# QinZiwen/VisionX-SLAM

Measured on AMD Instinct MI355X. Metric: ms/frame (feature-extract+match + BA solve), 640×480, 50 KF / 20k pts, lower is better.
Workload: dtype u8/i32 (FAST, pyramid, BRIEF), f32 (Harris, blur, angle), f64 (BA)

## Files before the change

### visionx-slam_amd/csrc/ba.hip

```cpp
#include <algorithm>
#include <cstddef>
#include <cstdlib>
#include <chrono>
#include <cmath>
#include <type_traits>
#include <cstring>
#include <unordered_map>
#include <unordered_set>
#include <vector>

#include "vx_internal.hpp"
#include "vx_ktrace.hpp"
#include "ba_common.hpp"
#include "ba_plan.hpp"
#include "dmap.hpp"

namespace vx {
namespace {

using namespace vx::ba;

constexpr int kPoseBlock = kBaPoseBlock;
constexpr int kNTerms = 29;
constexpr int kStride = kBaStride;
// ... 815 lines not shown
        double h[9];
        const D3 PO{lpos[3 * orec.y], lpos[3 * orec.y + 1], lpos[3 * orec.y + 2]};
        const bool ok = obs_terms<kFT <= kFTSmall>(a, PO, orec.x, ouv, kslot, kLdsStride, kslot + 8, kLdsStride,
                                                   kslot + 17, kLdsStride, h);
#pragma unroll
        for (int j = 0; j < 9; ++j) terms[j * kFT + tid] = h[j];
        tcount[tid] = (has_o && ok) ? 1 : 0;
        __syncthreads();
        if (own) {
            double hs[9] = {0, 0, 0, 0, 0, 0, 0, 0, 0};
            int obs = 0;
            for (int r = run.x; r < run.y; ++r) {
#pragma unroll
                for (int j = 0; j < 9; ++j) hs[j] += terms[j * kFT + r];
                obs += tcount[r];
            }
            asm volatile("" : "+v"(lslot));
            PL = lm_update(a, lslot, PL, hs, obs);
            if (kEcopy) f.lpos[base + tid] = make_double4(PL.x, PL.y, PL.z, 0.0);
            lpos[3 * tid] = PL.x;
            lpos[3 * tid + 1] = PL.y;
            lpos[3 * tid + 2] = PL.z;
        }
        __syncthreads();
    }
    FKT(4);
    if (!pose_next) return;
    int r = 0;
    FKT(6);
    for (int j = wv; j < n_ent; j += kFW) {
        const int4 e = s_ke[j];
        const int dst = s_kd[j];
        const int nr = (e.w - e.z + 63) >> 6;
        if (nr == 0) continue;
        const double* T = kslot + j * kLdsStride;
        const double* R = T + 8;
        const double* C = T + 17;
        double v[kStride];
#pragma unroll
        for (int t = 0; t < kStride; ++t) v[t] = 0.0;
        if constexpr (kCmp) {
            double* qw = qbuf + (size_t)wv * kQ * kQRec;
            int qh = 0, qn = 0;
            auto drain = [&](int n) {
                const int slot = (qh - qn + lane + kQ) & (kQ - 1);
                const double4 r0 = *reinterpret_cast<const double4*>(qw + (size_t)slot * kQRec);
                const double4 r1 = *reinterpret_cast<const double4*>(qw + (size_t)slot * kQRec + 4);
                const bool use = lane < n;
                pose_obs_terms(C, use ? r0.x : 0.0, use ? r0.y : 0.0, use ? r0.z : 1.0, use ? r0.w : 1.0,
                               use ? r1.x : 0.0, use ? r1.y : 0.0, use ? r1.z : 0.0, v);
                qn -= n;
            };
            for (int q = 0; q < nr; ++q, ++r) {
                const double2 uv = u0;
                const double4 P4 = p0;
                if (r + 1 < wrounds) {
                    u0 = f.pobs_uv[wstart + 64 * (r + 1) + lane];
                    p0 = f.pobs_p[wstart + 64 * (r + 1) + lane];
                }
                const bool valid = e.z + 64 * q + lane < e.w;
                const int code = (int)P4.w;
                const D3 P = code >= 0 ? D3{lpos[3 * code], lpos[3 * code + 1], lpos[3 * code + 2]} : D3{P4.x, P4.y, P4.z};
                const D3 pc = rt_apply(R, T + 4, P);
                const bool front = pc.z > 1e-6;
                const double inv_z = frcp(front ? pc.z : 1.0);
                const double e0 = uv.x - (C[0] * (pc.x * inv_z) + C[2]);
                const double e1 = uv.y - (C[1] * (pc.y * inv_z) + C[3]);
                const double e2 = e0 * e0 + e1 * e1;
                const bool ok = valid && front && !(e2 > a.max_err2);
                const double w = ok ? (e2 > a.huber2 ? a.huber * frsq(e2) : 1.0) : 0.0;
                v[27] = fma(w, e2, v[27]);
                v[28] += ok ? 1.0 : 0.0;
                const unsigned long long m = __ballot(ok);
                const int slot = ok ? ((qh + mbcnt_lo_hi(m)) & (kQ - 1)) : -1;
                if (ok) {
                    double4* rec = reinterpret_cast<double4*>(qw + (size_t)slot * kQRec);
                    rec[0] = make_double4(pc.x, pc.y, pc.z, inv_z);
                    rec[1] = make_double4(e0, e1, w, 0.0);
                }
                const int na = __popcll(m);
                qh = (qh + na) & (kQ - 1);
                qn += na;
                if (qn >= 64) {
                    __builtin_amdgcn_fence(__ATOMIC_RELEASE, "wavefront");
                    __builtin_amdgcn_wave_barrier();
                    __builtin_amdgcn_fence(__ATOMIC_ACQUIRE, "wavefront");
                    drain(64);
                }
            }
            if (qn > 0) {
                __builtin_amdgcn_fence(__ATOMIC_RELEASE, "wavefront");
                __builtin_amdgcn_wave_barrier();
                __builtin_amdgcn_fence(__ATOMIC_ACQUIRE, "wavefront");
                drain(qn);
            }
            __builtin_amdgcn_fence(__ATOMIC_RELEASE, "wavefront");
            __builtin_amdgcn_wave_barrier();
        } else {
        for (int q = 0; q < nr; ++q, ++r) {
            const double2 uv = u0;
            const double4 P4 = p0;
            if (r + 1 < wrounds) {
                int lim = f.padskip ? e.w - (e.z + 64 * (q + 1)) : 64;
                if (f.padskip && q + 1 >= nr) {
                    int jn = j + kFW;
                    int4 en = s_ke[jn < kFK ? jn : j];
                    while (jn < n_ent && ((en.w - en.z + 63) >> 6) == 0) {
                        jn += kFW;
                        en = s_ke[jn < kFK ? jn : j];
                    }
                    lim = en.w - en.z;
                }
                if (lane < lim) {
                    u0 = f.pobs_uv[wstart + 64 * (r + 1) + lane];
                    p0 = f.pobs_p[wstart + 64 * (r + 1) + lane];
                } else {
                    u0 = make_double2(0.0, 0.0);
                    p0 = make_double4(0.0, 0.0, 0.0, 0.0);
                }
            }
            const bool valid = e.z + 64 * q + lane < e.w;
            if (kFT <= kFTSmall || valid) {
                const int code = (int)P4.w;
                const D3 P = code >= 0 ? D3{lpos[3 * code], lpos[3 * code + 1], lpos[3 * code + 2]}
                                       : D3{P4.x, P4.y, P4.z};
                pose_obs_accum<kFT <= kFTSmall>(a, T, R, C, P, uv, v, valid);
            }
        }
        }
        if (j == wv) FKT(7);
        const double tot = wave_sum32(v);
        if (arow && (!kPro || f.apro)) {
            if ((lane & 1) == 0 && (lane >> 1) < kNTerms)
                unsafeAtomicAdd(arow + ((size_t)arow_wr(kPro, it) * f.n_kf + (e.x & 0x3fffffff)) * kStride + (lane >> 1),
                                tot);
            continue;
        }
        if ((lane & 1) == 0) part_out[(size_t)dst * kStride + (lane >> 1)] = (lane >> 1) < kNTerms ? tot : 0.0;
        if (lane == 54 || lane == 56)
            reinterpret_cast<double*>(f.costpart + (size_t)((it + 1) & 1) * f.n_part + dst)[(lane - 54) >> 1] = tot;
    }
    if (!kPro && it == 1) VX_KTW(8, 8);
    FKT(5);
}

typedef unsigned long long wgran;
struct WinArgs {
    wgran* part;
    wgran* stop;
    unsigned* hello;
    int* gen;
    int* fault;
    int bias;
};
constexpr long long kWinSpinTicks = 20'000'000;
constexpr int kWinGenMax = 0x7ffffff0;
constexpr int kWinSB = 8;
constexpr int kWinSStride = kStride + 1;
constexpr size_t win_lds(int ft) {
    return fused_lds(ft) + (size_t)kFK * kLdsStride * sizeof(double) + (size_t)ft * (16 + 16 + 12);
}
static_assert(win_lds(kFTSmall) <= 160 * 1024, "k_ba_win LDS exceeds gfx950's 160 KB per workgroup");
static_assert(kFK * kWinSStride <= 9 * kFTSmall, "k_ba_win stages the row sums in the landmark stage's terms");

__device__ __forceinline__ int ld_sc1(const int* p) { return __hip_atomic_load(p, __ATOMIC_RELAXED, __HIP_MEMORY_SCOPE_AGENT); }
__device__ __forceinline__ unsigned ld_sc1(const unsigned* p) {
    return __hip_atomic_load(p, __ATOMIC_RELAXED, __HIP_MEMORY_SCOPE_AGENT);
}
__device__ __forceinline__ wgran ld_sc1(const wgran* p) {
    return __hip_atomic_load(p, __ATOMIC_RELAXED, __HIP_MEMORY_SCOPE_AGENT);
}
__device__ __forceinline__ void st_gran2(wgran* g, double v, unsigned tag) {
    const unsigned long long u = (unsigned long long)__double_as_longlong(v), t = (unsigned long long)tag << 32;
    __hip_atomic_store(g, t | (u & 0xffffffffull), __ATOMIC_RELAXED, __HIP_MEMORY_SCOPE_AGENT);
    __hip_atomic_store(g + 1, t | (u >> 32), __ATOMIC_RELAXED, __HIP_MEMORY_SCOPE_AGENT);
}
__device__ __forceinline__ double gran2_value(wgran lo, wgran hi) {
    return __longlong_as_double((long long)((lo & 0xffffffffull) | (hi << 32)));
}
__device__ __forceinline__ bool win_spin_fail(int& k, long long t0, int* fault) {
    if ((++k & 15) == 0 && (ld_sc1(fault) || wall_clock64() - t0 > kWinSpinTicks)) {
        if ((threadIdx.x & 63) == 0) __hip_atomic_store(fault, 1, __ATOMIC_RELAXED, __HIP_MEMORY_SCOPE_AGENT);
        return true;
    }
    __builtin_amdgcn_s_sleep(1);
    return false;
}

template <int kFT>
__global__ __launch_bounds__(kFT) void k_ba_win(BAArgs a, FusedArgs f, WinArgs w) {
    constexpr int kFW = kFT / 64;
    static_assert(kFW >= 2, "k_ba_win: wave 1 runs the stop rule");
    __builtin_amdgcn_s_setprio(3);
    extern __shared__ __attribute__((aligned(16))) double fl[];
    __shared__ int4 s_ke[kFK];
    __shared__ int s_kd[kFK];
    __shared__ int s_act, s_fault;
    double* const ks0 = fl;
    double* terms = ks0 + 2 * kFK * kLdsStride;
    int* tcount = reinterpret_cast<int*>(terms + 9 * kFT);
    double* lpos = terms + 9 * kFT + kFT / 2;
    int4* s_orec = reinterpret_cast<int4*>(lpos + 3 * kFT);
    double2* s_ouv = reinterpret_cast<double2*>(s_orec + kFT);
    int* s_run = reinterpret_cast<int*>(s_ouv + kFT);
    const int tid = threadIdx.x, b = blockIdx.x, wv = tid >> 6, lane = tid & 63;
    const size_t base = (size_t)b * kFT;
    const int4* KE = f.kent + (size_t)b * kFK * 2;
    const int M = a.max_iter, nk = a.n_kf, nb = (int)gridDim.x;
    const int nslot = nk * f.maxl;
    const int gen = w.gen[0];
    const unsigned tag = (unsigned)gen + 1u;
    if (gen < 0 || gen >= kWinGenMax) {
        if (tid == 0) __hip_atomic_store(w.fault, 1, __ATOMIC_RELAXED, __HIP_MEMORY_SCOPE_AGENT);
        return;
    }
    if (tid == 0) __hip_atomic_store(w.hello + b, tag, __ATOMIC_RELAXED, __HIP_MEMORY_SCOPE_AGENT);
    const int wvu = __builtin_amdgcn_readfirstlane(wv);
    const int4 B = f.blk[(size_t)b * (1 + kFW / 2)];
    const int4 WB = f.blk[(size_t)b * (1 + kFW / 2) + 1 + (wvu >> 1)];
    int4 ke = make_int4(-1, 0, 0, 0);
    int kd = -1;
    if (tid < kFK) {
        ke = KE[2 * tid];
        kd = KE[2 * tid + 1].x;
    }
    const int4 orec0 = f.lobs_rec[base + tid];
    const double2 ouv0 = f.lobs_uv[base + tid];
    const int lslot0 = f.lm_slot[base + tid];
    const int2 run0 = f.lm_run[base + tid];
    D3 PL;
    {
        const double* P = a.lm_pos0 + 4 * (size_t)lslot0;
        PL = {P[0], P[1], P[2]};
    }
    const int wstart = (wvu & 1) ? WB.z : WB.x, wrounds = (wvu & 1) ? WB.w : WB.y;
    double2 u0 = make_double2(0, 0);
    double4 p0 = make_double4(0, 0, 0, 0);
    auto first_round = [&] {
        if (wrounds > 0) {
            u0 = f.pobs_uv[wstart + lane];
            p0 = f.pobs_p[wstart + lane];
        }
    };
    first_round();
    double ev[13];
    const int row = ke.x & 0x3fffffff;
    if (tid < kFK && ke.x >= 0) {
#pragma unroll
        for (int j = 0; j < 8; ++j) ev[j] = a.kf_pose0[8 * (size_t)row + j];
#pragma unroll
        for (int j = 0; j < 4; ++j) ev[8 + j] = a.kf_intr[4 * row + j];
        ev[12] = (double)a.kf_flags[row];
    }
    if (b == 0 && tid < 16) {
        a.state->cost[tid] = 0.0;
        a.state->obs[tid] = 0;
    }
    const int n_lm = B.x, n_ob = B.y, n_ent = B.z;
    const bool has_o = tid < n_ob, own = tid < n_lm;
    lpos[3 * tid] = PL.x;
    lpos[3 * tid + 1] = PL.y;
    lpos[3 * tid + 2] = PL.z;
    s_orec[tid] = orec0;
    s_ouv[tid] = ouv0;
    s_run[3 * tid] = run0.x;
    s_run[3 * tid + 1] = run0.y;
    s_run[3 * tid + 2] = lslot0;
    if (tid < kFK) {
        s_ke[tid] = ke;
        s_kd[tid] = kd;
    }
    if (tid == 0) s_fault = 0;
    if (tid < kFK && ke.x >= 0) {
        double Rm[9];
        rot_from_quat(ev, Rm);
        double* sl = ks0 + (kFK + tid) * kLdsStride;
        double* sl0 = ks0 + tid * kLdsStride;
#pragma unroll
        for (int j = 0; j < 8; ++j) sl[j] = ev[j];
#pragma unroll
        for (int j = 0; j < 9; ++j) sl[8 + j] = Rm[j];
#pragma unroll
        for (int j = 0; j < 4; ++j) sl[17 + j] = sl0[17 + j] = ev[8 + j];
        sl[21] = sl0[21] = ev[12];
    }
    __syncthreads();

    auto pose_stage = [&](int itn) {
        int r = 0;
        wgran* const Pn = w.part + (size_t)itn * (nslot + 1) * (2 * kStride);
        const double* const kslot = ks0 + ((itn - 1) & 1) * kFK * kLdsStride;
        for (int j = wv; j < n_ent; j += kFW) {
            const int4 e = s_ke[j];
            const int nr = (e.w - e.z + 63) >> 6;
            if (nr == 0) continue;
            const double* T = kslot + j * kLdsStride;
            const double* Rr = T + 8;
            const double* C = T + 17;
            double v[kStride];
#pragma unroll
            for (int t = 0; t < kStride; ++t) v[t] = 0.0;
            for (int q = 0; q < nr; ++q, ++r) {
                const double2 uv = u0;
                const double4 P4 = p0;
                if (r + 1 < wrounds) {
                    int lim = e.w - (e.z + 64 * (q + 1));
                    if (q + 1 >= nr) {
                        int jn = j + kFW;
                        int4 en = s_ke[jn < kFK ? jn : j];
                        while (jn < n_ent && ((en.w - en.z + 63) >> 6) == 0) {
                            jn += kFW;
                            en = s_ke[jn < kFK ? jn : j];
                        }
                        lim = en.w - en.z;
                    }
                    if (lane < lim) {
                        u0 = f.pobs_uv[wstart + 64 * (r + 1) + lane];
                        p0 = f.pobs_p[wstart + 64 * (r + 1) + lane];
                    } else {
                        u0 = make_double2(0.0, 0.0);
                        p0 = make_double4(0.0, 0.0, 0.0, 0.0);
                    }
                }
                const bool valid = e.z + 64 * q + lane < e.w;
                const int code = (int)P4.w;
                const D3 P = code >= 0 ? D3{lpos[3 * code], lpos[3 * code + 1], lpos[3 * code + 2]} : D3{P4.x, P4.y, P4.z};
                pose_obs_accum<true>(a, T, Rr, C, P, uv, v, valid);
            }
            const double tot = wave_sum32(v);
            const int kdj = s_kd[j];
            if ((lane & 1) == 0 && (lane >> 1) < kNTerms && kdj >= 0)
                st_gran2(Pn + ((size_t)kdj * kStride + (lane >> 1)) * 2, tot, tag);
        }
    };
    auto hello_sweep = [&]() -> int {
        const long long t0 = wall_clock64();
        for (int spins = 0;;) {
            bool ok = true;
            for (int q = lane; q < nb; q += 64) ok &= ld_sc1(w.hello + q) == tag;
            if (__all(ok)) return 1;
            if (win_spin_fail(spins, t0, w.fault)) return -1;
        }
    };
    double last = 1.7976931348623157e308;
    auto decide_issue = [&](int ip, wgran (&d)[4]) {
        const wgran* const g = w.stop + ((size_t)ip * nk + (lane < nk ? lane : 0)) * 4;
#pragma unroll
        for (int i = 0; i < 4; ++i) d[i] = ld_sc1(g + i);
    };
    auto decide = [&](int ip, const wgran (&d)[4]) -> int {
        const wgran* const sp = w.stop + (size_t)ip * nk * 4;
        const long long t0 = wall_clock64();
        int spins = 0;
        double tot = 0.0, cn = 0.0;
        for (int q0 = 0; q0 < nk; q0 += 64) {
            const bool live = q0 + lane < nk;
            const wgran* const g = sp + (size_t)(live ? q0 + lane : 0) * 4;
            wgran c0 = d[0], c1 = d[1], n0 = d[2], n1 = d[3];
            for (bool first = q0 == 0;; first = false) {
                if (!first) c0 = ld_sc1(g), c1 = ld_sc1(g + 1), n0 = ld_sc1(g + 2), n1 = ld_sc1(g + 3);
                const bool ok = !live || ((unsigned)(c0 >> 32) == tag && (unsigned)(c1 >> 32) == tag &&
                                          (unsigned)(n0 >> 32) == tag && (unsigned)(n1 >> 32) == tag);
                if (__all(ok)) break;
                if (win_spin_fail(spins, t0, w.fault)) return -1;
            }
            __builtin_amdgcn_fence(__ATOMIC_ACQUIRE, "wavefront");
            tot += live ? gran2_value(c0, c1) : 0.0;
            cn += live ? gran2_value(n0, n1) : 0.0;
        }
#pragma unroll
        for (int m = 32; m > 0; m >>= 1) {
            tot += __shfl_xor(tot, m, 64);
            cn += __shfl_xor(cn, m, 64);
        }
        const int tobs = (int)cn;
        const bool stop = tobs == 0 || fabs(last - tot) < 1e-6 * last;
        if (!stop) last = tot;
        if (b == 0 && lane == 0) {
            BAState* s = a.state;
            if (ip < 16) {
                s->cost[ip] = tot;
                s->obs[ip] = tobs;
            }
            s->iterations = ip + 1;
            s->last_cost = last;
            if (!stop && ip + 1 < M)
                s->active[ip + 1] = 1;
            else
                for (int k = ip + 1; k <= M; ++k) s->active[k] = 0;
        }
        return stop ? 0 : 1;
    };

    VX_KT(0);
    pose_stage(0);
    if (wv == 0) VX_KT(15);
    for (int it = 0; it < M; ++it) {
        double* const kslot = ks0 + (it & 1) * kFK * kLdsStride;
        const double* const kprev = ks0 + ((it + 1) & 1) * kFK * kLdsStride;
        wgran dgr[4] = {0, 0, 0, 0};
        if (wv == 1 && it > 0) decide_issue(it - 1, dgr);
        {
            const int h = lane >> 5, t = lane & 31;
            const wgran* const Pi = w.part + (size_t)it * (nslot + 1) * (2 * kStride);
            double* const stage = terms;
            const long long t0 = wall_clock64();
            int spins = 0;
            bool okw = true;
            __builtin_amdgcn_s_setprio(0);
            for (int j = wv; j < n_ent && okw; j += kFW) {
                const int4 e = s_ke[j];
                if (e.x < 0) continue;
                const int erow = e.x & 0x3fffffff;
                const int ns = e.y + (erow == 0 ? w.bias : 0);
                double acc = 0.0;
                for (int s0 = 0; s0 < ns && okw; s0 += 2 * kWinSB) {
                    wgran g0[kWinSB], g1[kWinSB];
                    unsigned have = 0;
#pragma unroll
                    for (int i = 0; i < kWinSB; ++i) {
                        g0[i] = g1[i] = 0;
                        if (!(s0 + 2 * i + h < ns && t < kNTerms)) have |= 1u << i;
                    }
                    for (;;) {
#pragma unroll
                        for (int i = 0; i < kWinSB; ++i)
                            if (!((have >> i) & 1)) {
                                const int q = s0 + 2 * i + h;
                                const int slot = q < e.y ? erow * f.maxl + q : nslot;
                                const wgran* g = Pi + ((size_t)slot * kStride + t) * 2;
                                g0[i] = ld_sc1(g);
                                g1[i] = ld_sc1(g + 1);
                            }
#pragma unroll
                        for (int i = 0; i < kWinSB; ++i)
                            if (!((have >> i) & 1) && (unsigned)(g0[i] >> 32) == tag && (unsigned)(g1[i] >> 32) == tag)
                                have |= 1u << i;
                        if (__all(have == (1u << kWinSB) - 1)) break;
                        if (win_spin_fail(spins, t0, w.fault)) {
                            okw = false;
                            break;
                        }
                    }
                    __builtin_amdgcn_fence(__ATOMIC_ACQUIRE, "wavefront");
#pragma unroll
                    for (int i = 0; i < kWinSB; ++i) {
                        const bool live = s0 + 2 * i + h < ns && t < kNTerms;
                        const double v = live ? gran2_value(g0[i], g1[i]) : 0.0;
                        const double vo = __shfl(v, t + 32, 64);
                        acc += v;
                        acc += vo;
                    }
                }
                if (lane < kNTerms) stage[j * kWinSStride + lane] = acc;
                if (okw && (e.x & (1 << 30)) && (lane == 27 || lane == 28))
                    st_gran2(w.stop + ((size_t)it * nk + erow) * 4 + (lane - 27) * 2, acc, tag);
            }
            __builtin_amdgcn_s_setprio(3);
// ... 245 lines not shown
        const double* src = kf_pose + (size_t)(st->iterations & 1) * n_kf * 8 + (size_t)8 * i;
        for (int j = 0; j < 7; ++j) map_pose[(size_t)7 * kf_map[i] + j] = src[j];
    }
    if (i < n_opt)
        for (int j = 0; j < 3; ++j) map_pos[(size_t)3 * lm_map[i] + j] = lm_pos[(size_t)4 * i + j];
}
}

int alloc_run_buffers(vx_ctx* c, vx_ba_plan* p) {
    const size_t nk = (size_t)p->n_kf;
    VX_HIP(c, p->kf_pose.ensure(nk * 2 * 8 * sizeof(double)));
    VX_HIP(c, p->kf_rot.ensure(nk * 9 * sizeof(double)));
    VX_HIP(c, p->kf_part.ensure(nk * p->n_split * kStride * sizeof(double)));
    VX_HIP(c, p->kf_cost.ensure(nk * 2 * sizeof(double)));
    VX_HIP(c, p->lm_pos.ensure((size_t)std::max(p->n_lm, 1) * 4 * sizeof(double)));
    VX_HIP(c, p->state.ensure(sizeof(BAState)));
    VX_HIP(c, hipMemsetAsync(p->state.p, 0, sizeof(BAState), c->stream));
    return VX_OK;
}

namespace {
template <class B>
void swap_buf(B& a, B& b) {
    std::swap(a.p, b.p);
    std::swap(a.bytes, b.bytes);
}
void adopt_buffers(vx_ba_plan* dst, vx_ba_plan* src) {
#define VX_SWAP_BUF(b) swap_buf(dst->b, src->b);
    VX_PLAN_BUFFERS(VX_SWAP_BUF)
#undef VX_SWAP_BUF
}
constexpr size_t kMaxPlanHusks = 4;
}

vx_ba_plan* plan_new(vx_ctx* c) {
    auto* p = new vx_ba_plan();
    p->c = c;
    if (!c) return p;
    if (!c->plan_husks.empty()) {
        vx_ba_plan* h = c->plan_husks.back();
        c->plan_husks.pop_back();
        adopt_buffers(p, h);
        delete h;
    }
    c->plan_live.push_back(p);
    return p;
}

int plan_fault_injected(vx_ctx* c) {
    const char* e = getenv("VX_TEST_FAIL_PLAN");
    return (e && e[0] == '1') ? set_error(c, VX_ERR_STATE, "plan build failed ($VX_TEST_FAIL_PLAN)") : VX_OK;
}

void plan_pool_release(vx_ctx* c) {
    for (vx_ba_plan* h : c->plan_husks) delete h;
    c->plan_husks.clear();
    for (vx_ba_plan* p : c->plan_live) p->c = nullptr;
    c->plan_live.clear();
}

bool fused_eligible(const vx_ba_plan* p) {
    if (p->status != 0 || p->global_poses || p->n_kf > kMaxKfLds || p->n_opt <= 0) return false;
    if (const char* e = getenv("VX_BA_FUSED"))
        if (e[0] == '0') return false;
    return true;
}

bool ba_persist() {
    const char* e = getenv("VX_BA_PERSIST");
    return !(e && e[0] == '0');
}

bool ba_atomic_rows() {
    const char* e = getenv("VX_BA_ATOMIC_ROWS");
    return !(e && e[0] == '0');
}

int fused_threads(vx_ctx* c, int64_t n_lobs, int* cap) {
    if (!c->n_cus) c->n_cus = std::max(vx_device_cus(c->device), 1);
    int ft = n_lobs > (int64_t)c->n_cus * (kFTSmall - 16) ? kFTLarge : kFTSmall;
    if (const char* e = getenv("VX_BA_FUSED_THREADS")) {
        const int v = atoi(e);
        ft = v == kFTLarge ? kFTLarge : v == kFTNarrow ? kFTNarrow : kFTSmall;
    }
    *cap = ft;
    if (const char* e = getenv("VX_BA_FUSED_CAP")) *cap = std::min(ft, std::max(64, atoi(e)));
    return ft;
}

size_t fused_offsets(int nb, int ft, size_t n_pp, FusedOffsets& F) {
    const size_t n_lp = (size_t)nb * ft;
    size_t at = 0;
    auto take = [&](size_t bytes) {
        const size_t o = at;
        at += (bytes + 255) & ~(size_t)255;
        return o;
    };
    F.blk = take((size_t)nb * fused_blk_ints(ft) * 4);
    F.lm_slot = take(n_lp * 4);
    F.lm_run = take(n_lp * 8);
    F.lobs_rec = take(n_lp * 16);
    F.kent = take((size_t)nb * kFK * 32);
    F.lobs_src = take(n_lp * 4);
    F.pobs_src = take(std::max<size_t>(n_pp, 1) * 4);
    F.pobs_code = take(std::max<size_t>(n_pp, 1) * 4);
    return at;
}

int fused_finish(vx_ctx* c, vx_ba_plan* p, int nb, int ft, int maxl, size_t n_pp, int stop_b) {
    const FusedOffsets& F = p->f_off;
    const size_t n_lp = (size_t)nb * ft;
    const uint8_t* T = p->f_tab.as<uint8_t>();
    VX_HIP(c, p->f_lobs_uv.ensure(n_lp * sizeof(double2)));
    VX_HIP(c, p->f_pobs_uv.ensure(std::max<size_t>(n_pp, 1) * sizeof(double2)));
    VX_HIP(c, p->f_pobs_p.ensure(std::max<size_t>(n_pp, 1) * sizeof(double4)));
    hipLaunchKernelGGL(k_fused_gather, dim3((unsigned)((std::max(n_lp, n_pp) + 255) / 256)), dim3(256), 0, c->stream,
                       reinterpret_cast<const int*>(T + F.lobs_src), (int)n_lp, (const double2*)p->lobs_uv.as<double2>(),
                       p->f_lobs_uv.as<double2>(), reinterpret_cast<const int*>(T + F.pobs_src),
                       reinterpret_cast<const int*>(T + F.pobs_code), (int)n_pp, (const double2*)p->pobs_uv.as<double2>(),
                       (const double*)p->lm_pos0.as<double>(), p->f_pobs_uv.as<double2>(), p->f_pobs_p.as<double4>());
    VX_LAUNCH_CHECK(c, "k_fused_gather");
    VX_HIP(c, p->f_lpos.ensure(n_lp * sizeof(double4)));
    VX_HIP(c, p->f_epose.ensure((size_t)nb * kFK * 16 * sizeof(double)));
    const size_t part_bytes = 2 * (size_t)p->n_kf * maxl * kStride * sizeof(double);
    VX_HIP(c, p->f_part.ensure(part_bytes));
    if (p->shard_count > 1) VX_HIP(c, p->f_rowpart.ensure((size_t)p->n_kf * kStride * sizeof(double)));
    VX_HIP(c, hipMemsetAsync(p->f_part.p, 0, part_bytes, c->stream));
    const size_t cost_bytes = 2 * (size_t)p->n_kf * maxl * sizeof(double2);
    VX_HIP(c, p->f_costpart.ensure(cost_bytes));
    VX_HIP(c, hipMemsetAsync(p->f_costpart.p, 0, cost_bytes, c->stream));
    p->f_atomic = p->shard_count <= 1 && ft <= kFTSmall && ba_atomic_rows();
    if (p->f_atomic) {
        const size_t ab = 4 * (size_t)p->n_kf * kStride * sizeof(double);
        VX_HIP(c, p->f_arow.ensure(ab));
        VX_HIP(c, hipMemsetAsync(p->f_arow.p, 0, ab, c->stream));
    }
    p->f_persist = false;
    p->win_off = false;
    if (!c->n_cus) c->n_cus = std::max(vx_device_cus(c->device), 1);
    if (p->f_atomic && ft == kFTSmall && nb <= c->n_cus && p->opt.max_iterations >= 1 &&
        p->opt.max_iterations <= kMaxIter && ba_persist()) {
        const size_t M = (size_t)p->opt.max_iterations, nk = (size_t)p->n_kf;
        size_t at = 0;
        auto take = [&](size_t bytes) {
            const size_t o = at;
            at += (bytes + 255) & ~(size_t)255;
            return o;
        };
        p->win_part_off = take(M * (nk * (size_t)maxl + 1) * kStride * 2 * sizeof(wgran));
        p->win_stop_off = take(M * nk * 4 * sizeof(wgran));
        p->win_hello_off = take((size_t)nb * sizeof(unsigned));
        p->win_gen_off = take(sizeof(int));
        p->win_bias = getenv("VX_BA_WIN_TEST_FAULT") ? 1 : 0;
        VX_HIP(c, p->f_win.ensure(at));
        VX_HIP(c, hipMemsetAsync(p->f_win.p, 0, at, c->stream));
        p->f_persist = true;
    }
    p->f_stop_b = stop_b;
    p->f_blocks = nb;
    p->f_maxl = maxl;
    p->f_threads = ft;
    p->f_npp = n_pp;
    p->fused = true;
    return VX_OK;
}

int build_fused(vx_ctx* c, vx_ba_plan* p, const std::vector<int>& kptr, const std::vector<int>& plm,
                const std::vector<int>& lptr, const std::vector<int>& lkf) {
    p->fused = false;
    if (!fused_eligible(p)) return VX_OK;
    const int nk = p->n_kf, n_opt = p->n_opt, n_pose = kptr[nk];
    static const bool timing = getenv("VX_PLAN_TIMING") != nullptr;
    using clk = std::chrono::steady_clock;
    const auto t_start = clk::now();
    double t_ph[16] = {0};
    auto lap = [&](int i) { t_ph[i] = std::chrono::duration<double, std::milli>(clk::now() - t_start).count(); };
    std::vector<int> pkf(n_pose);
    for (int k = 0; k < nk; ++k)
        for (int o = kptr[k]; o < kptr[k + 1]; ++o) pkf[o] = k;
    std::vector<int> pp(n_opt + 1, 0), pidx;
    for (int o = 0; o < n_pose; ++o)
        if (plm[o] < n_opt) ++pp[plm[o] + 1];
    for (int q = 0; q < n_opt; ++q) pp[q + 1] += pp[q];
    pidx.resize(pp[n_opt]);
    {
        std::vector<int> w(pp.begin(), pp.end() - 1);
        for (int o = 0; o < n_pose; ++o)
            if (plm[o] < n_opt) pidx[w[plm[o]]++] = o;
    }
    lap(3);
    std::vector<int> key(n_opt, nk), order(n_opt);
    for (int q = 0; q < n_opt; ++q) {
        int k0 = nk;
        for (int o = lptr[q]; o < lptr[q + 1]; ++o) k0 = std::min(k0, lkf[o]);
        for (int i = pp[q]; i < pp[q + 1]; ++i) k0 = std::min(k0, pkf[pidx[i]]);
        key[q] = k0;
    }
    {
        std::vector<int> kc(nk + 2, 0);
        for (int q = 0; q < n_opt; ++q) ++kc[key[q] + 1];
        for (int k = 0; k <= nk; ++k) kc[k + 1] += kc[k];
        for (int q = 0; q < n_opt; ++q) order[kc[key[q]]++] = q;
    }
    lap(4);
    std::vector<int> uk_ptr(n_opt + 1, 0), uk;
    uk.reserve((size_t)lptr[n_opt] + pidx.size());
    {
        std::vector<int> seen(nk, -1);
        for (int q = 0; q < n_opt; ++q) {
            for (int o = lptr[q]; o < lptr[q + 1]; ++o)
                if (seen[lkf[o]] != q) {
                    seen[lkf[o]] = q;
                    uk.push_back(lkf[o]);
                }
            for (int i = pp[q]; i < pp[q + 1]; ++i)
                if (seen[pkf[pidx[i]]] != q) {
                    seen[pkf[pidx[i]]] = q;
                    uk.push_back(pkf[pidx[i]]);
                }
            uk_ptr[q + 1] = (int)uk.size();
        }
    }
    lap(5);
    int cap = 0;
    const int ft = fused_threads(c, lptr[n_opt], &cap);
    std::vector<std::vector<int>> K(1), LM(1);
    std::vector<int> stamp(nk, -1);
    int n_l = 0, n_o = 0;
    for (int idx = 0; idx < n_opt; ++idx) {
        const int q = order[idx], cnt = lptr[q + 1] - lptr[q];
        if (cnt > ft) return VX_OK;
        int cur = (int)K.size() - 1;
        int nn = 0;
        for (int u = uk_ptr[q]; u < uk_ptr[q + 1]; ++u) nn += stamp[uk[u]] != cur;
        if (n_l > 0 && (n_l + 1 > cap || n_o + cnt > cap || (int)K[cur].size() + nn > kFK)) {
            K.emplace_back();
            LM.emplace_back();
            ++cur;
            n_l = n_o = 0;
            nn = uk_ptr[q + 1] - uk_ptr[q];
        }
        if (nn > kFK) return VX_OK;
        for (int u = uk_ptr[q]; u < uk_ptr[q + 1]; ++u)
            if (stamp[uk[u]] != cur) {
                stamp[uk[u]] = cur;
                K[cur].push_back(uk[u]);
            }
        LM[cur].push_back(q);
        ++n_l;
        n_o += cnt;
    }
    const int nb = (int)K.size();
    if (nb > kFusedMaxGroups) return VX_OK;
    const int fw = ft / 64;
    lap(0);
    std::vector<int> owner(nk, -1);
    for (int b = 0; b < nb; ++b)
        for (int k : K[b])
            if (owner[k] < 0) owner[k] = b;
    for (int k = 0; k < nk; ++k)
        if (owner[k] < 0) {
            owner[k] = 0;
            K[0].push_back(k);
        }
    if ((int)K[0].size() > kFK) return VX_OK;
    for (auto& v : K) std::sort(v.begin(), v.end());
    lap(6);
    std::vector<int> lm_blk(n_opt), lm_loc(n_opt);
    for (int b = 0; b < nb; ++b)
        for (int i = 0; i < (int)LM[b].size(); ++i) {
            lm_blk[LM[b][i]] = b;
            lm_loc[LM[b][i]] = i;
        }
    std::vector<int> po_ptr(nb + 1, 0), po(n_pose), po_blk(n_pose);
    for (int o = 0; o < n_pose; ++o) {
        po_blk[o] = plm[o] < n_opt ? lm_blk[plm[o]] : owner[pkf[o]];
        ++po_ptr[po_blk[o] + 1];
    }
    for (int b = 0; b < nb; ++b) po_ptr[b + 1] += po_ptr[b];
    {
        std::vector<int> w(po_ptr.begin(), po_ptr.end() - 1);
        for (int o = 0; o < n_pose; ++o) po[w[po_blk[o]]++] = o;
    }
    const int kBlkInts = fused_blk_ints(ft);
    lap(7);
    std::vector<int> ent_beg((size_t)nb * kFK, 0), ent_end((size_t)nb * kFK, 0);
    size_t n_pp = 0;
    for (int b = 0; b < nb; ++b) {
        int i = po_ptr[b];
        for (int j = 0; j < (int)K[b].size(); ++j) {
            ent_beg[(size_t)b * kFK + j] = i;
            while (i < po_ptr[b + 1] && pkf[po[i]] == K[b][j]) ++i;
            ent_end[(size_t)b * kFK + j] = i;
            n_pp += (size_t)(i - ent_beg[(size_t)b * kFK + j] + 63) / 64 * 64;
        }
        if (i != po_ptr[b + 1]) return set_error(c, VX_ERR_STATE, "fused layout: pose observations out of keyframe order");
    }
    std::vector<int> epos((size_t)nb * kFK, -1), n_pos(nb, 0);
    for (int b = 0; b < nb; ++b) {
        int rounds[kFK];
        const int ne = (int)K[b].size();
        for (int j = 0; j < ne; ++j)
            rounds[j] = (ent_end[(size_t)b * kFK + j] - ent_beg[(size_t)b * kFK + j] + 63) / 64;
        n_pos[b] = fused_place_entries(rounds, ne, &epos[(size_t)b * kFK]);
    }
    FusedOffsets& F = p->f_off;
// ... 294 lines not shown
    const uint8_t* T = p->f_tab.as<uint8_t>();
    f.blk = reinterpret_cast<const int4*>(T + p->f_off.blk);
    f.lm_slot = reinterpret_cast<const int*>(T + p->f_off.lm_slot);
    f.lm_run = reinterpret_cast<const int2*>(T + p->f_off.lm_run);
    f.lobs_uv = p->f_lobs_uv.as<double2>();
    f.lobs_rec = reinterpret_cast<const int4*>(T + p->f_off.lobs_rec);
    f.kent = reinterpret_cast<const int4*>(T + p->f_off.kent);
    f.pobs_uv = p->f_pobs_uv.as<double2>();
    f.pobs_p = p->f_pobs_p.as<double4>();
    f.part = p->f_part.as<double>();
    f.maxl = p->f_maxl;
    f.n_part = p->n_kf * p->f_maxl;
    f.rowpart = p->shard_count > 1 ? p->f_rowpart.as<double>() : nullptr;
    f.costpart = p->f_costpart.as<double2>();
    f.stop_b = p->f_stop_b;
    f.lpos = p->f_lpos.as<double4>();
    f.epose = p->f_epose.as<double>();
    f.arow = p->f_atomic && p->shard_count <= 1 ? p->f_arow.as<double>() : nullptr;
    f.n_kf = p->n_kf;
    f.apro = p->opt.max_iterations >= 2;
    static const int drow_env = [] {
        const char* e = getenv("VX_BA_DROW");
        return e && e[0] == '0' ? 0 : 1;
    }();
    f.drow = drow_env;
    static const int padskip_env = [] {
        const char* e = getenv("VX_BA_PADSKIP");
        return e && e[0] == '0' ? 0 : 1;
    }();
    f.padskip = padskip_env;
    return f;
}

bool ba_compact() {
    static const bool on = [] {
        const char* e = std::getenv("VX_BA_COMPACT");
        return e && e[0] == '1';
    }();
    return on;
}

template <int kFT>
int fused_launch_t(vx_ctx* c, vx_ba_plan* p, const BAArgs& a, const FusedArgs& f, int it) {
    constexpr int lds = (int)fused_lds(kFT);
    constexpr int lds_c = (int)fused_lds_cmp(kFTSmall);
    static std::atomic<uint64_t> d0{0}, d1{0}, d2{0};
    VX_HIP(c, lds_attr_once(c->device, reinterpret_cast<const void*>(&k_ba_iter<true, kFT>), lds, d0));
    VX_HIP(c, lds_attr_once(c->device, reinterpret_cast<const void*>(&k_ba_iter<false, kFT>), lds, d1));
    VX_HIP(c, lds_attr_once(c->device, reinterpret_cast<const void*>(&k_ba_iter<false, kFTSmall, true>), lds_c, d2));
    if (it < 0)
        VX_HIP(c, launch(c, kStBaPrologue, k_ba_iter<true, kFT>, dim3(p->f_blocks), dim3(kFT), (uint32_t)lds, c->stream,
                         a, f, -1));
    else if (kFT == kFTSmall && ba_compact())
        VX_HIP(c, launch(c, kStBaIter, k_ba_iter<false, kFTSmall, true>, dim3(p->f_blocks), dim3(kFTSmall),
                         (uint32_t)lds_c, c->stream, a, f, it));
    else
        VX_HIP(c, launch(c, kStBaIter, k_ba_iter<false, kFT>, dim3(p->f_blocks), dim3(kFT), (uint32_t)lds, c->stream,
                         a, f, it));
    return VX_OK;
}
int fused_launch(vx_ctx* c, vx_ba_plan* p, const BAArgs& a, const FusedArgs& f, int it) {
    if (p->f_threads == kFTLarge) return fused_launch_t<kFTLarge>(c, p, a, f, it);
    if (p->f_threads == kFTNarrow) return fused_launch_t<kFTNarrow>(c, p, a, f, it);
    return fused_launch_t<kFTSmall>(c, p, a, f, it);
}
int fused_row_sum(vx_ctx* c, vx_ba_plan* p, int it) {
    const int n = p->n_kf * kStride;
    ProfScope ps(c, kStBaPoseSum);
    hipLaunchKernelGGL(k_row_sum, dim3((n + 255) / 256), dim3(256), 0, c->stream,
                       (const double*)(p->f_part.as<double>() + (size_t)(it & 1) * p->n_kf * p->f_maxl * kStride),
                       p->n_kf, p->f_maxl, p->f_rowpart.as<double>());
    VX_LAUNCH_CHECK(c, "k_row_sum");
    return VX_OK;
}

size_t peer_len(const vx_ba_plan* p) { return (size_t)p->n_kf * kStride; }
int peer_publish(vx_ctx* c, vx_ba_plan* p, int it, unsigned long long gen) {
    const size_t len = peer_len(p);
    double* blk = static_cast<double*>(p->peer_mem);
    if (!blk) return set_error(c, VX_ERR_STATE, "peer reduction: no block of its own");
    hipLaunchKernelGGL(k_peer_publish, dim3(1), dim3(1024), 0, c->stream,
                       (const double*)(p->f_part.as<double>() + (size_t)(it & 1) * p->n_kf * p->f_maxl * kStride), p->n_kf,
                       p->f_maxl, blk + (gen & 1) * len, reinterpret_cast<unsigned long long*>(blk + 2 * len), gen);
    VX_LAUNCH_CHECK(c, "k_peer_publish");
    return VX_OK;
}
int peer_gather(vx_ctx* c, vx_ba_plan* p, unsigned long long gen) {
    const size_t len = peer_len(p);
    const int n = (int)p->peer_base.size();
    PeerPtrs pp{};
    if (n < 1 || n > kMaxPeers) return set_error(c, VX_ERR_STATE, "peer reduction: %d ranks", n);
    for (int r = 0; r < n; ++r) {
        const double* b = static_cast<const double*>(p->peer_base[r]);
        if (!b) return set_error(c, VX_ERR_STATE, "peer reduction: rank %d's block is not mapped", r);
        pp.rows[r] = b;
        pp.flag[r] = reinterpret_cast<const unsigned long long*>(b + 2 * len);
    }
    hipLaunchKernelGGL(k_peer_gather, dim3(1), dim3(1024), 0, c->stream, pp, n, (int)len, (int)((gen & 1) * len), gen,
                       p->f_rowpart.as<double>(), reinterpret_cast<int*>(p->state.as<uint8_t>() + offsetof(BAState, fault)));
    VX_LAUNCH_CHECK(c, "k_peer_gather");
    return VX_OK;
}
size_t peer_bytes(const vx_ba_plan* p) { return ((2 * peer_len(p) + 8) * sizeof(double) + 4095) & ~(size_t)4095; }

#ifndef VX_NO_RCCL
int peer_setup(vx_ctx* c, vx_ba_plan* p) {
    const int n = p->shard_count, me = p->shard_rank;
    if (n > kMaxPeers) return set_error(c, VX_ERR_INVALID, "$VX_BA_PEER: at most %d ranks", kMaxPeers);
    if (c->nranks != n || c->rank != me)
        return set_error(c, VX_ERR_INVALID, "$VX_BA_PEER: shard %d of %d on communicator rank %d of %d", me, n, c->rank,
                         c->nranks);
    const size_t bytes = peer_bytes(p);
    VX_HIP(c, hipExtMallocWithFlags(&p->peer_mem, bytes, hipDeviceMallocUncached));
    VX_HIP(c, hipMemsetAsync(p->peer_mem, 0, bytes, c->stream));
    hipIpcMemHandle_t h;
    VX_HIP(c, hipIpcGetMemHandle(&h, p->peer_mem));
    DevBuf d;
    VX_HIP(c, d.ensure((size_t)n * sizeof h));
    VX_HIP(c, hipMemcpyAsync(d.as<uint8_t>() + (size_t)me * sizeof h, &h, sizeof h, hipMemcpyHostToDevice, c->stream));
    ncclResult_t r = ncclAllGather(d.as<uint8_t>() + (size_t)me * sizeof h, d.p, sizeof h, ncclUint8, c->comm, c->stream);
    if (r != ncclSuccess) return set_error(c, VX_ERR_COMM, "ncclAllGather (peer handles): %s", ncclGetErrorString(r));
    std::vector<hipIpcMemHandle_t> all(n);
    VX_HIP(c, hipMemcpyAsync(all.data(), d.p, (size_t)n * sizeof h, hipMemcpyDeviceToHost, c->stream));
    VX_HIP(c, hipStreamSynchronize(c->stream));
    p->peer_base.assign(n, nullptr);
    for (int q = 0; q < n; ++q) {
        if (q == me) {
            p->peer_base[q] = p->peer_mem;
            continue;
        }
        void* ptr = nullptr;
        VX_HIP(c, hipIpcOpenMemHandle(&ptr, all[q], hipIpcMemLazyEnablePeerAccess));
        p->peer_opened.push_back(ptr);
        p->peer_base[q] = ptr;
    }
    p->peer = true;
    return VX_OK;
}
#endif

bool peer_requested() {
    const char* e = getenv("VX_BA_PEER");
    return e && e[0] == '1';
}

WinArgs make_win_args(vx_ba_plan* p) {
    uint8_t* W = p->f_win.as<uint8_t>();
    WinArgs w{};
    w.part = reinterpret_cast<wgran*>(W + p->win_part_off);
    w.stop = reinterpret_cast<wgran*>(W + p->win_stop_off);
    w.hello = reinterpret_cast<unsigned*>(W + p->win_hello_off);
    w.gen = reinterpret_cast<int*>(W + p->win_gen_off);
    w.bias = p->win_bias;
    w.fault = reinterpret_cast<int*>(p->state.as<uint8_t>() + offsetof(BAState, fault));
    return w;
}

bool win_active(const vx_ba_plan* p) { return p->fused && p->f_persist && !p->win_off && p->shard_count <= 1; }

int plan_run_fused(vx_ctx* c, vx_ba_plan* p) {
    const BAArgs a = make_args(p);
    const FusedArgs f = make_fused_args(p);
    int rc;
    if ((rc = reset_if_no_iterations(c, p, a))) return rc;
    if (p->opt.max_iterations == 0) return VX_OK;
    if (win_active(p)) {
        constexpr int lds = (int)win_lds(kFTSmall);
        static std::atomic<uint64_t> dw{0};
        VX_HIP(c, lds_attr_once(c->device, reinterpret_cast<const void*>(&k_ba_win<kFTSmall>), lds, dw));
        VX_HIP(c, launch(c, kStBaWin, k_ba_win<kFTSmall>, dim3(p->f_blocks), dim3(kFTSmall), (uint32_t)lds, c->stream,
                         a, f, make_win_args(p)));
        return VX_OK;
    }
    if ((rc = fused_launch(c, p, a, f, -1))) return rc;
#ifndef VX_NO_RCCL
    if (p->shard_count > 1 && !p->peer && peer_requested() && (rc = peer_setup(c, p))) return rc;
#endif
    for (int it = 0; it < p->opt.max_iterations; ++it) {
        if (p->shard_count > 1 && p->peer) {
            const unsigned long long gen = ++p->peer_gen;
            if ((rc = peer_publish(c, p, it, gen)) || (rc = peer_gather(c, p, gen))) return rc;
        } else if (p->shard_count > 1) {
#ifndef VX_NO_RCCL
            if ((rc = fused_row_sum(c, p, it))) return rc;
            ProfScope ps(c, kStBaAllreduce);
            ncclResult_t r = ncclAllReduce(p->f_rowpart.p, p->f_rowpart.p, (size_t)p->n_kf * kStride, ncclDouble, ncclSum,
                                           c->comm, c->stream);
            if (r != ncclSuccess) return set_error(c, VX_ERR_COMM, "ncclAllReduce: %s", ncclGetErrorString(r));
#else
            return set_error(c, VX_ERR_COMM, "built without RCCL");
#endif
        }
        if ((rc = fused_launch(c, p, a, f, it))) return rc;
    }
    return VX_OK;
}

int plan_run(vx_ctx* c, vx_ba_plan* p) {
    if (p->status != 0) {
        p->ran = true;
        return VX_OK;
    }
    const bool sharded = p->shard_count > 1;
    int rc;
    if (sharded) {
#ifndef VX_NO_RCCL
        if (!c->comm || c->nranks != p->shard_count || c->rank != p->shard_rank)
            return set_error(c, VX_ERR_STATE, "sharded plan needs vx_comm_init(%d ranks)", p->shard_count);
        if ((rc = shard_kernel_choice(c, p))) return rc;
#else
        return set_error(c, VX_ERR_COMM, "built without RCCL");
#endif
    }
    if (p->fused && (!sharded || p->fused_all)) {
        rc = plan_run_fused(c, p);
        if (!rc) p->ran = true;
        return rc;
    }
    if (!sharded && !p->choice_made) {
        p->lds_poses = choose_lds_poses(p, p->n_lm_blocks, p->max_lm_obs);
        p->choice_made = true;
    }
    const BAArgs a = make_args(p);
    if ((rc = reset_if_no_iterations(c, p, a))) return rc;
    for (int it = 0; it < p->opt.max_iterations; ++it) {
        if ((rc = pose_stage(c, p, a, it))) return rc;
#ifndef VX_NO_RCCL
        if (sharded) {
            ProfScope ps(c, kStBaAllreduce);
            ncclResult_t r = ncclAllReduce(p->kf_part.p, p->kf_part.p, (size_t)p->n_kf * p->n_split * kStride, ncclDouble,
                                           ncclSum, c->comm, c->stream);
            if (r != ncclSuccess) return set_error(c, VX_ERR_COMM, "ncclAllReduce: %s", ncclGetErrorString(r));
        }
#endif
        if ((rc = landmark_stage(c, p, a, it, p->lds_poses))) return rc;
    }
    p->ran = true;
    return VX_OK;
}

}

size_t ba_state_bytes() { return sizeof(BAState); }

size_t ba_state_iter_offset() { return offsetof(BAState, iterations); }

void ba_state_to_stats(const void* host_state, vx_ba_stats* s) {
    const BAState& hs = *static_cast<const BAState*>(host_state);
    s->iterations = hs.iterations;
    for (int i = 0; i < 16; ++i) {
        s->cost[i] = hs.cost[i];
        s->obs[i] = hs.obs[i];
    }
}

int ba_run_dyn(vx_ctx* c, const DynPlan& d) {
    BAArgs a{};
    a.n_kf = d.n_kf;
    a.n_opt = 0;
    a.n_lm = 0;
    a.min_pose_obs = d.opt.min_pose_observations;
    a.min_point_obs = d.opt.min_point_observations;
    a.max_iter = d.opt.max_iterations;
    a.huber = d.opt.huber_delta;
    a.max_err = d.opt.max_reproj_error;
    a.huber2 = a.huber * a.huber;
    a.max_err2 = a.max_err * a.max_err;
    a.kf_pose0 = d.kf_pose0;
    a.kf_pose = d.kf_pose;
    a.kf_intr = d.kf_intr;
    a.kf_rot = d.kf_rot;
    a.kf_flags = d.kf_flags;
    a.kf_obs_ptr = d.kf_obs_ptr;
    a.kf_part = d.kf_part;
    a.n_split = d.n_split;
    a.kf_cost = d.kf_cost;
    a.lm_pos0 = d.lm_pos0;
    a.lm_pos = d.lm_pos;
    a.pobs_uv = d.pobs_uv;
    a.pobs_lm = d.pobs_lm;
    a.lobs_ptr = d.lobs_ptr;
    a.lobs_kf = d.lobs_kf;
    a.lobs_lm = d.lobs_lm;
    a.lm_blk = d.lm_blk;
    a.lobs_uv = d.lobs_uv;
    a.state = static_cast<BAState*>(d.state);
    a.dyn = d.dyn;
    const size_t lds = (size_t)d.n_kf * kLdsStride * sizeof(double) + (size_t)kLmBlock * (9 * sizeof(double) + sizeof(int));
    if (lds > 64 * 1024) {
        static std::atomic<uint64_t> done{0};
        VX_HIP(c, lds_attr_once(c->device, reinterpret_cast<const void*>(&k_landmark_solve), 160 * 1024, done));
    }
    for (int it = 0; it < d.opt.max_iterations; ++it) {
        VX_HIP(c, launch(c, kStBaPose, k_pose_kf, dim3(d.n_kf * d.n_split), dim3(kPoseBlock), 0, c->stream, a, it));
        VX_HIP(c, launch(c, kStBaLandmark, k_landmark_solve, dim3(d.grid_blocks), dim3(kLmBlock), (uint32_t)lds,
                         c->stream, a, it));
    }
    return VX_OK;
}

namespace {
constexpr int kMaxEmuShards = 16;
struct PartPtrs {
    double* p[kMaxEmuShards];
};
__global__ void k_sum_parts(PartPtrs parts, int n, long long len) {
    const long long i = (long long)blockIdx.x * blockDim.x + threadIdx.x;
    if (i >= len) return;
    double s = parts.p[0][i];
    for (int r = 1; r < n; ++r) s += parts.p[r][i];
    for (int r = 0; r < n; ++r) parts.p[r][i] = s;
}

}
}

using namespace vx;

VX_KT_EXPORT(vx_ktrace_read_ba);

namespace vx {
int lean_optimize_view(vx_ctx* c, vx_map_view* v, uint64_t ref, int has_ref, const vx_ba_options& o, vx_ba_stats* st,
                       bool* fallback);
}
// ... 434 lines not shown
```

### visionx-slam_amd/csrc/ba_plan.hpp

```cpp
#pragma once
#include <cstdint>
#include <vector>

#include "vx_internal.hpp"

struct FusedOffsets {
    size_t blk = 0, lm_slot = 0, lm_run = 0, lobs_rec = 0, kent = 0, lobs_src = 0, pobs_src = 0, pobs_code = 0;
};

struct vx_ba_plan {
    vx_ctx* c = nullptr;
    vx_ba_options opt{};
    int status = 1;
    int shard_rank = 0, shard_count = 1;
    int n_window_kf = 0, n_landmarks_global = 0;
    int n_kf = 0, n_opt = 0, n_lm = 0;
    int64_t n_pose_obs = 0, n_lm_obs = 0;
    std::vector<int> kf_map_idx, lm_map_idx;
    int n_split = 1;
    vx::DevBuf kf_pose0, kf_pose, kf_intr, kf_rot, kf_flags, kf_obs_ptr, kf_part, kf_cost, lm_pos0, lm_pos,
        pobs_uv, pobs_lm, lobs_ptr, lobs_kf, lobs_lm, lm_blk, lobs_uv, state;
    int n_lm_blocks = 1;
    int max_lm_obs = 0;
    bool choice_made = false;
    bool lds_poses = true;
    bool ran = false;
    vx::OwnedGraph graph;
    bool graph_eager = false;
    vx::DevBuf kf_map_dev, lm_map_dev;
    bool from_dmap = false;
    bool global_poses = false;
    bool fused = false;
    bool fused_all = false;
    int f_blocks = 0, f_maxl = 0, f_threads = 512;
    vx::DevBuf f_tab, f_lobs_uv, f_pobs_uv, f_pobs_p, f_part;
    vx::DevBuf f_rowpart;
    vx::DevBuf f_lpos, f_epose;
    vx::DevBuf f_costpart;
    vx::DevBuf f_arow;
    bool f_atomic = false;
    vx::DevBuf f_win;
    bool f_persist = false, win_off = false;
    size_t win_part_off = 0, win_stop_off = 0, win_hello_off = 0, win_gen_off = 0;
    int win_bias = 0;
    int f_stop_b = 0;
    vx::PinnedBuf f_stage;
    vx::PinnedBuf fetch_host;
    bool peer = false;
    void* peer_mem = nullptr;
    std::vector<void*> peer_base, peer_opened;
    unsigned long long peer_gen = 0;
    FusedOffsets f_off;
    size_t f_npp = 0;
};

struct vx_dmap;

#define VX_PLAN_BUFFERS(X)                                                                              \
    X(kf_pose0) X(kf_pose) X(kf_intr) X(kf_rot) X(kf_flags) X(kf_obs_ptr) X(kf_part) X(kf_cost) X(lm_pos0) \
    X(lm_pos) X(pobs_uv) X(pobs_lm) X(lobs_ptr) X(lobs_kf) X(lobs_lm) X(lm_blk) X(lobs_uv) X(state)       \
    X(kf_map_dev) X(lm_map_dev) X(f_tab) X(f_lobs_uv) X(f_pobs_uv) X(f_pobs_p) X(f_part) X(f_rowpart)    \
    X(f_stage) X(f_lpos) X(f_epose) X(f_costpart) X(f_arow) X(f_win) X(fetch_host)

namespace vx {
vx_ba_plan* plan_new(vx_ctx* c);
#ifndef VX_BA_POSE_BLOCK
#define VX_BA_POSE_BLOCK 512
#endif
#ifndef VX_BA_MAX_SPLIT
#define VX_BA_MAX_SPLIT 4
#endif
constexpr int kBaPoseBlock = VX_BA_POSE_BLOCK;
constexpr int kBaLmBlock = 512;
constexpr int kBaMaxSplit = VX_BA_MAX_SPLIT;

inline int ba_split(int64_t mx, int shard_count) {
    const int64_t per = (int64_t)kBaPoseBlock * (shard_count > 1 ? shard_count : 1);
    const int64_t s = (mx + per - 1) / per;
    return (int)(s < 1 ? 1 : (s > kBaMaxSplit ? kBaMaxSplit : s));
}

int alloc_run_buffers(vx_ctx* c, vx_ba_plan* p);
int build_fused(vx_ctx* c, vx_ba_plan* p, const std::vector<int>& kf_obs_ptr, const std::vector<int>& plm,
                const std::vector<int>& lptr, const std::vector<int>& lkf);
int build_fused_device(vx_ctx* c, vx_ba_plan* p);
constexpr int kBaFusedK = 64;
constexpr int kFusedMaxGroups = 8192;
constexpr int kBaFTSmall = 512, kBaFTLarge = 1024;
constexpr int kBaFTNarrow = 256;
constexpr int kBaStride = 32;
constexpr int kBaMaxKfLds = 448;
bool fused_eligible(const vx_ba_plan* p);
int fused_threads(vx_ctx* c, int64_t n_lobs, int* cap);
size_t fused_offsets(int nb, int ft, size_t n_pp, FusedOffsets& F);
inline int fused_blk_ints(int ft) { return 4 * (1 + ft / 64 / 2); }
int fused_finish(vx_ctx* c, vx_ba_plan* p, int nb, int ft, int maxl, size_t n_pp, int stop_b);
__host__ __device__ inline int fused_place_entries(const int* rounds, int n, int* pos) {
    int load[4] = {0, 0, 0, 0}, cnt[4] = {0, 0, 0, 0}, n_pos = 0;
    unsigned long long done = 0;
    for (int it = 0; it < n; ++it) {
        int j = -1;
        for (int i = 0; i < n; ++i)
            if (!((done >> i) & 1) && (j < 0 || rounds[i] > rounds[j])) j = i;
        done |= 1ull << j;
        int s = -1;
        for (int q = 0; q < 4; ++q)
            if (cnt[q] < 16 && (s < 0 || load[q] < load[s] || (load[q] == load[s] && cnt[q] < cnt[s]))) s = q;
        pos[j] = s + 4 * cnt[s];
        ++cnt[s];
        load[s] += rounds[j];
        n_pos = pos[j] + 1 > n_pos ? pos[j] + 1 : n_pos;
    }
    return n_pos;
}

__host__ __device__ inline long long fused_stop_key(int max_wave_rounds, int n_ent, int b) {
    return ((long long)(max_wave_rounds * 64 + n_ent) << 32) | (unsigned)b;
}
int build_plan_device(vx_ctx* c, const vx_map_view* m, uint64_t ref_kf_id, int has_ref, vx_ba_plan* p);
int build_plan_dmap(vx_ctx* c, vx_dmap* m, uint64_t ref_kf_id, int has_ref, vx_ba_plan* p);
std::vector<int> pack_lm_blocks(const std::vector<int>& lptr, int n_opt, int* max_cnt);

enum : int { kDynNOpt = 0, kDynNLm, kDynBlocks, kDynStatus, kDynPoseObs, kDynLmObs, kDynGlobal, kDynMaxObs,
             kDynNFixed,
             kDynSbaOo, kDynSbaPairs, kDynSbaMaxObs, kDynSbaBlocks, kDynSbaLmBlocks, kDynInts = 16 };
struct DynPlan {
    int n_kf = 0, n_split = 1, grid_blocks = 0;
    vx_ba_options opt{};
    const double* kf_pose0 = nullptr;
    double* kf_pose = nullptr;
    const double* kf_intr = nullptr;
    double* kf_rot = nullptr;
    const int* kf_flags = nullptr;
    const int* kf_obs_ptr = nullptr;
    double* kf_part = nullptr;
    double* kf_cost = nullptr;
    const double* lm_pos0 = nullptr;
    double* lm_pos = nullptr;
    const double2* pobs_uv = nullptr;
    const int* pobs_lm = nullptr;
    const int* lobs_ptr = nullptr;
    const int* lobs_kf = nullptr;
    const int* lobs_lm = nullptr;
    const int* lm_blk = nullptr;
    const double2* lobs_uv = nullptr;
    void* state = nullptr;
    const int* dyn = nullptr;
};
int ba_run_dyn(vx_ctx* c, const DynPlan& d);
size_t ba_state_bytes();
size_t ba_state_iter_offset();
void ba_state_to_stats(const void* host_state, vx_ba_stats* s);
constexpr int kBaStrideDoubles = 32;
}
```

Baseline: 0.05100.

## Cache pose-stage observation records in spare LDS across BA iterations

The persistent windowed BA kernel now preloads as many per-wave pose-observation rounds (uv and point records) as fit in the unused LDS budget. The pose stage then reads those rounds from LDS on every iteration and falls back to global loads only for rounds beyond the cached count. The cross-block stop-rule batch size also becomes a macro and moves from 8 to 10. In exchange the kernel uses much more dynamic LDS and pays an up-front copy at launch, and the cache size can be overridden through an environment variable.

```diff
diff --git a/visionx-slam_amd/csrc/ba.hip b/visionx-slam_amd/csrc/ba.hip
--- a/visionx-slam_amd/csrc/ba.hip
+++ b/visionx-slam_amd/csrc/ba.hip
@@ -991,15 +991,25 @@
     int* gen;
     int* fault;
     int bias;
+    int rec_rounds;
 };
 constexpr long long kWinSpinTicks = 20'000'000;
 constexpr int kWinGenMax = 0x7ffffff0;
-constexpr int kWinSB = 8;
+#ifndef VX_WIN_SB
+#define VX_WIN_SB 10
+#endif
+constexpr int kWinSB = VX_WIN_SB;
+static_assert(kWinSB >= 1 && kWinSB <= 16, "k_ba_win: the sweep's `have` mask and its register budget");
 constexpr int kWinSStride = kStride + 1;
 constexpr size_t win_lds(int ft) {
     return fused_lds(ft) + (size_t)kFK * kLdsStride * sizeof(double) + (size_t)ft * (16 + 16 + 12);
 }
-static_assert(win_lds(kFTSmall) <= 160 * 1024, "k_ba_win LDS exceeds gfx950's 160 KB per workgroup");
+constexpr size_t kWinRecRound = 3 * 64 * sizeof(double2);
+constexpr size_t kWinStaticLds = 2048;
+constexpr int kWinRecRoundsMax = (int)((160 * 1024 - kWinStaticLds - win_lds(kFTSmall)) / kWinRecRound);
+static_assert(win_lds(kFTSmall) % 16 == 0, "k_ba_win: the pose-stage records in LDS are 16-byte aligned");
+static_assert(win_lds(kFTSmall) + kWinRecRoundsMax * kWinRecRound + kWinStaticLds <= 160 * 1024,
+              "k_ba_win LDS exceeds gfx950's 160 KB per workgroup");
 static_assert(kFK * kWinSStride <= 9 * kFTSmall, "k_ba_win stages the row sums in the landmark stage's terms");
 
 __device__ __forceinline__ int ld_sc1(const int* p) { return __hip_atomic_load(p, __ATOMIC_RELAXED, __HIP_MEMORY_SCOPE_AGENT); }
@@ -1042,6 +1052,8 @@
     int4* s_orec = reinterpret_cast<int4*>(lpos + 3 * kFT);
     double2* s_ouv = reinterpret_cast<double2*>(s_orec + kFT);
     int* s_run = reinterpret_cast<int*>(s_ouv + kFT);
+    static_assert(sizeof(s_ke) + sizeof(s_kd) + 2 * sizeof(int) <= kWinStaticLds, "k_ba_win: static LDS");
+    double2* const s_rec = reinterpret_cast<double2*>(reinterpret_cast<char*>(fl) + win_lds(kFT));
     const int tid = threadIdx.x, b = blockIdx.x, wv = tid >> 6, lane = tid & 63;
     const size_t base = (size_t)b * kFT;
     const int4* KE = f.kent + (size_t)b * kFK * 2;
@@ -1073,15 +1085,48 @@
         PL = {P[0], P[1], P[2]};
     }
     const int wstart = (wvu & 1) ? WB.z : WB.x, wrounds = (wvu & 1) ? WB.w : WB.y;
+    int pre = 0;
+#pragma unroll
+    for (int q = 0; q < kFW / 2; ++q) {
+        const int4 X = f.blk[(size_t)b * (1 + kFW / 2) + 1 + q];
+        pre += (2 * q < wvu ? X.y : 0) + (2 * q + 1 < wvu ? X.w : 0);
+    }
+    const int rl = min(max(w.rec_rounds - pre, 0), wrounds);
+    double2* const wrec = s_rec + (size_t)pre * (3 * 64) + lane;
     double2 u0 = make_double2(0, 0);
     double4 p0 = make_double4(0, 0, 0, 0);
+    auto lds_round = [&](int r) {
+        const double2* const R = wrec + (size_t)r * (3 * 64);
+        const double2 xy = R[64], zc = R[128];
+        u0 = R[0];
+        p0 = make_double4(xy.x, xy.y, zc.x, zc.y);
+    };
     auto first_round = [&] {
-        if (wrounds > 0) {
+        if (rl > 0) {
+            lds_round(0);
+        } else if (wrounds > 0) {
             u0 = f.pobs_uv[wstart + lane];
             p0 = f.pobs_p[wstart + lane];
         }
     };
-    first_round();
+    if (rl == 0) first_round();
+    for (int r0 = 0; r0 < rl; r0 += 4) {
+        const int ra = r0, rb = min(r0 + 1, rl - 1), rc = min(r0 + 2, rl - 1), rd = min(r0 + 3, rl - 1);
+        const double2 ua = f.pobs_uv[wstart + 64 * ra + lane], ub = f.pobs_uv[wstart + 64 * rb + lane];
+        const double2 uc = f.pobs_uv[wstart + 64 * rc + lane], ud = f.pobs_uv[wstart + 64 * rd + lane];
+        const double4 pa = f.pobs_p[wstart + 64 * ra + lane], pb = f.pobs_p[wstart + 64 * rb + lane];
+        const double4 pc = f.pobs_p[wstart + 64 * rc + lane], pd = f.pobs_p[wstart + 64 * rd + lane];
+        auto put = [&](int r, const double2& u, const double4& p) {
+            double2* const R = wrec + (size_t)r * (3 * 64);
+            R[0] = u;
+            R[64] = make_double2(p.x, p.y);
+            R[128] = make_double2(p.z, p.w);
+        };
+        put(ra, ua, pa);
+        put(rb, ub, pb);
+        put(rc, uc, pc);
+        put(rd, ud, pd);
+    }
     double ev[13];
     const int row = ke.x & 0x3fffffff;
     if (tid < kFK && ke.x >= 0) {
@@ -1124,6 +1169,7 @@
         sl[21] = sl0[21] = ev[12];
     }
     __syncthreads();
+    if (rl > 0) first_round();
 
     auto pose_stage = [&](int itn) {
         int r = 0;
@@ -1142,7 +1188,9 @@
             for (int q = 0; q < nr; ++q, ++r) {
                 const double2 uv = u0;
                 const double4 P4 = p0;
-                if (r + 1 < wrounds) {
+                if (r + 1 < rl) {
+                    lds_round(r + 1);
+                } else if (r + 1 < wrounds) {
                     int lim = e.w - (e.z + 64 * (q + 1));
                     if (q + 1 >= nr) {
                         int jn = j + kFW;
@@ -1694,6 +1742,9 @@
         p->win_hello_off = take((size_t)nb * sizeof(unsigned));
         p->win_gen_off = take(sizeof(int));
         p->win_bias = getenv("VX_BA_WIN_TEST_FAULT") ? 1 : 0;
+        p->win_rec_rounds = kWinRecRoundsMax;
+        if (const char* e = getenv("VX_BA_WIN_LDS_ROUNDS"))
+            p->win_rec_rounds = std::min(kWinRecRoundsMax, std::max(0, atoi(e)));
         VX_HIP(c, p->f_win.ensure(at));
         VX_HIP(c, hipMemsetAsync(p->f_win.p, 0, at, c->stream));
         p->f_persist = true;
@@ -2294,6 +2345,7 @@
     w.hello = reinterpret_cast<unsigned*>(W + p->win_hello_off);
     w.gen = reinterpret_cast<int*>(W + p->win_gen_off);
     w.bias = p->win_bias;
+    w.rec_rounds = p->win_rec_rounds;
     w.fault = reinterpret_cast<int*>(p->state.as<uint8_t>() + offsetof(BAState, fault));
     return w;
 }
@@ -2307,11 +2359,13 @@
     if ((rc = reset_if_no_iterations(c, p, a))) return rc;
     if (p->opt.max_iterations == 0) return VX_OK;
     if (win_active(p)) {
-        constexpr int lds = (int)win_lds(kFTSmall);
+        constexpr int lds_max = (int)(win_lds(kFTSmall) + kWinRecRoundsMax * kWinRecRound);
+        const WinArgs w = make_win_args(p);
+        if (w.rec_rounds < 0 || w.rec_rounds > kWinRecRoundsMax) return set_error(c, VX_ERR_STATE, "k_ba_win: LDS rounds");
+        const uint32_t lds = (uint32_t)(win_lds(kFTSmall) + (size_t)w.rec_rounds * kWinRecRound);
         static std::atomic<uint64_t> dw{0};
-        VX_HIP(c, lds_attr_once(c->device, reinterpret_cast<const void*>(&k_ba_win<kFTSmall>), lds, dw));
-        VX_HIP(c, launch(c, kStBaWin, k_ba_win<kFTSmall>, dim3(p->f_blocks), dim3(kFTSmall), (uint32_t)lds, c->stream,
-                         a, f, make_win_args(p)));
+        VX_HIP(c, lds_attr_once(c->device, reinterpret_cast<const void*>(&k_ba_win<kFTSmall>), lds_max, dw));
+        VX_HIP(c, launch(c, kStBaWin, k_ba_win<kFTSmall>, dim3(p->f_blocks), dim3(kFTSmall), lds, c->stream, a, f, w));
         return VX_OK;
     }
     if ((rc = fused_launch(c, p, a, f, -1))) return rc;
diff --git a/visionx-slam_amd/csrc/ba_plan.hpp b/visionx-slam_amd/csrc/ba_plan.hpp
--- a/visionx-slam_amd/csrc/ba_plan.hpp
+++ b/visionx-slam_amd/csrc/ba_plan.hpp
@@ -43,6 +43,7 @@
     bool f_persist = false, win_off = false;
     size_t win_part_off = 0, win_stop_off = 0, win_hello_off = 0, win_gen_off = 0;
     int win_bias = 0;
+    int win_rec_rounds = 0;
     int f_stop_b = 0;
     vx::PinnedBuf f_stage;
     vx::PinnedBuf fetch_host;
```

Result: slower. 0.05160 (+1.2%).
